# gabrielspmoreira/chameleon_recsys

Hardware: NVIDIA H100
Metric: NAR train interactions/sec (higher is better)
Workload: dtype f32 (wgmma: bf16x3 (error-compensated) forward, single-pass TF32 backward; fp32 accumulate)

## Files before the change

### chameleon_recsys_b200/_lib.py

```python
from __future__ import annotations

import ctypes as C
import os
from typing import Optional

HERE = os.path.dirname(os.path.abspath(__file__))
LIB_PATH = os.path.join(HERE, 'libnar_b200.so')

NAR_MAX_SEGMENTS = 24
NAR_MAX_SRC = 16
NAR_MAX_COLS = 1024

ACT_NONE, ACT_LEAKY, ACT_TANH = 0, 1, 2


class NarError(RuntimeError):
    pass


class Segment(C.Structure):
    _fields_ = [('kind', C.c_int32), ('col', C.c_int32), ('width', C.c_int32), ('card', C.c_int32),
                ('src', C.c_int32), ('ld', C.c_int32), ('table', C.c_void_p), ('grad', C.c_void_p)]


# ... 51 lines not shown


class NoveltyReg(C.Structure):
    _fields_ = [('factor', C.c_float), ('log_base', C.c_float), ('pop_norm', C.c_void_p), ('cand_ids', C.c_void_p),
                ('loss_nov', C.c_void_p)]


class GemmEpilogue(C.Structure):
    _fields_ = [('bias', C.c_void_p), ('act', C.c_int32), ('dact', C.c_int32), ('aux', C.c_void_p),
                ('ld_aux', C.c_int64), ('accumulate', C.c_int32), ('split_k', C.c_int32),
                ('precision', C.c_int32), ('b_lo', C.c_void_p), ('b_bf16', C.c_void_p), ('ld_bf16', C.c_int64),
                ('a_scale', C.c_void_p), ('ld_a_scale', C.c_int64), ('a_scale_group', C.c_int64),
                ('pred', C.c_void_p), ('d_pred', C.c_void_p), ('ld_pred', C.c_int64), ('pred_group', C.c_int64),
                ('d_bias', C.c_void_p), ('car_pp', C.c_void_p), ('car_pc', C.c_void_p), ('car_pi', C.c_void_p), ('car_pos_idx', C.c_void_p),
                ('car_neg_uidx', C.c_void_p), ('car_dpp', C.c_void_p), ('car_dpc', C.c_void_p), ('car_dpi', C.c_void_p),
                ('ld_car', C.c_int64), ('car_k', C.c_int64)]


_lib: Optional[C.CDLL] = None

i64, i32, f32, vp, u64, u32 = C.c_int64, C.c_int32, C.c_float, C.c_void_p, C.c_uint64, C.c_uint32

_SIGNATURES = {
    'nar_abi_version': (C.c_int, []),
    'nar_abi_struct_size': (C.c_int, [C.c_int]),
    'nar_status_string': (C.c_char_p, [C.c_int]),
    'nar_ctx_create': (C.c_int, [C.c_int, C.POINTER(vp)]),
    'nar_ctx_destroy': (C.c_int, [vp]),
    'nar_gather_features': (C.c_int, [vp, C.POINTER(FeaturePlanC), vp, vp, C.POINTER(RowLayout), vp, vp, vp, vp]),
    'nar_gather_features_bwd': (C.c_int, [vp, C.POINTER(FeaturePlanC), vp, vp, C.POINTER(RowLayout), vp, vp, vp, vp, vp, vp]),
    'nar_build_base_rows': (C.c_int, [vp, i64, vp, vp, vp, vp, i64, vp, i64, vp, vp, vp]),
# ... 120 lines not shown
```

### chameleon_recsys_b200/csrc/gemm_wgmma.cu

```cuda
#include "common.cuh"
#include <cuda_bf16.h>
#include <stdlib.h>
#include <string.h>
#include <type_traits>

namespace nar {
namespace gemm {

constexpr int BM = 128;
constexpr int BN = 128;
constexpr int BK = 32;
constexpr int TILE_BYTES = 128 * BK * 4;
constexpr int NUM_THREADS = 256;
constexpr int EPI_LD = BN + 4;

constexpr int EXT_SCALE_SMEM = 1, EXT_SCALE_GMEM = 2, EXT_PROD_BWD = 3, EXT_CAR_BWD = 4, EXT_TRANS_D = 5;
constexpr int SC_ROWS_K = 32, SC_ROWS_MN = 8;
constexpr int SC_BYTES = 4096;
static_assert(SC_ROWS_K * BK * 4 == SC_BYTES && SC_ROWS_MN * BM * 4 == SC_BYTES, "a_scale slice per stage");

template <int MODE, bool B_MN, int SC = 0> struct Cfg {
  static constexpr bool SPLIT3 = MODE == 1 || MODE == 2;
  static constexpr bool BLO = MODE == 2;
  static constexpr bool PREP = B_MN || SPLIT3;
  static constexpr bool PREP_TILES = SPLIT3;
  static constexpr int STAGE_BYTES = TILE_BYTES * (BLO ? 3 : 2);
  static constexpr int CTAS_PER_SM = PREP_TILES ? 1 : 2;
  static constexpr int STAGES = (BLO || !PREP_TILES) ? 3 : 4;
  static constexpr int PREP_TILE_BYTES = PREP_TILES ? TILE_BYTES * 2 : 0;
  static constexpr int PREP_BYTES = 2 * PREP_TILE_BYTES;
  static constexpr int SC_OFF = STAGES * STAGE_BYTES + PREP_BYTES;
  static constexpr int BAR_OFF = SC_OFF + STAGES * SC;
  static constexpr int SMEM_BYTES = BAR_OFF + 64 + 1024;
  static_assert(STAGES * STAGE_BYTES >= BM * EPI_LD * 4, "the epilogue stages the accumulators in the operand ring");
  static_assert(SMEM_BYTES <= 227 * 1024, "227 KB of shared memory per block");
  static_assert(CTAS_PER_SM * (SMEM_BYTES + 1024) <= 228 * 1024, "228 KB of shared memory per SM (1 KB reserved per block)");
};

struct Params {
  int64_t M, N, K;
  float* D; int64_t ldd;
  const float* bias;
  const float* aux; int64_t ld_aux;
  int act, dact, accumulate;
  int k_tiles_per_split;
  int n_tiles;
  const float* a_scale; int64_t ld_a_scale, a_rows, a_cols; uint32_t group;
  const float* pred; float* d_pred; float* d_bias; int64_t ld_pred, n_pos; int pos_per_tile;
  const float *car_pp, *car_pc, *car_pi; const int32_t *car_pos_idx, *car_neg_uidx;
// ... 26 lines not shown

__device__ __forceinline__ void tma_load_2d(uint32_t smem_dst, const CUtensorMap* map, uint64_t* bar, int c0, int c1) {
  asm volatile(
      "cp.async.bulk.tensor.2d.shared::cluster.global.mbarrier::complete_tx::bytes [%0], [%1, {%3, %4}], [%2];"
      ::"r"(smem_dst), "l"(reinterpret_cast<uint64_t>(map)), "r"(smem_u32(bar)), "r"(c0), "r"(c1)
      : "memory");
}
__device__ __forceinline__ void tma_prefetch_desc(const CUtensorMap* map) {
  asm volatile("prefetch.tensormap [%0];" ::"l"(reinterpret_cast<uint64_t>(map)) : "memory");
}

__device__ __forceinline__ void wgmma_fence() { asm volatile("wgmma.fence.sync.aligned;" ::: "memory"); }
__device__ __forceinline__ void wgmma_commit() { asm volatile("wgmma.commit_group.sync.aligned;" ::: "memory"); }
template <int N>
__device__ __forceinline__ void wgmma_wait() { asm volatile("wgmma.wait_group.sync.aligned %0;" ::"n"(N) : "memory"); }
__device__ __forceinline__ void fence_acc(float (&d)[64]) {
#pragma unroll
  for (int i = 0; i < 64; ++i) asm volatile("" : "+f"(d[i])::"memory");
}

__device__ __forceinline__ void wgmma_tf32(float (&d)[64], const uint32_t (&a)[4], uint64_t bdesc) {
  asm volatile(
      "{\n\t.reg .pred p;\n\tsetp.ne.b32 p, 1, 0;\n\t"
      "wgmma.mma_async.sync.aligned.m64n128k8.f32.tf32.tf32 "
      "{%0, %1, %2, %3, %4, %5, %6, %7, %8, %9, %10, %11, %12, %13, %14, %15, "
      "%16, %17, %18, %19, %20, %21, %22, %23, %24, %25, %26, %27, %28, %29, %30, %31, "
      "%32, %33, %34, %35, %36, %37, %38, %39, %40, %41, %42, %43, %44, %45, %46, %47, "
      "%48, %49, %50, %51, %52, %53, %54, %55, %56, %57, %58, %59, %60, %61, %62, %63}, "
      "{%64, %65, %66, %67}, %68, p, 1, 1;\n\t}"
      : "+f"(d[0]), "+f"(d[1]), "+f"(d[2]), "+f"(d[3]), "+f"(d[4]), "+f"(d[5]), "+f"(d[6]), "+f"(d[7]),
        "+f"(d[8]), "+f"(d[9]), "+f"(d[10]), "+f"(d[11]), "+f"(d[12]), "+f"(d[13]), "+f"(d[14]), "+f"(d[15]),
        "+f"(d[16]), "+f"(d[17]), "+f"(d[18]), "+f"(d[19]), "+f"(d[20]), "+f"(d[21]), "+f"(d[22]), "+f"(d[23]),
        "+f"(d[24]), "+f"(d[25]), "+f"(d[26]), "+f"(d[27]), "+f"(d[28]), "+f"(d[29]), "+f"(d[30]), "+f"(d[31]),
// ... 9 lines not shown
      "{\n\t.reg .pred p;\n\tsetp.ne.b32 p, 1, 0;\n\t"
      "wgmma.mma_async.sync.aligned.m64n128k16.f32.bf16.bf16 "
      "{%0, %1, %2, %3, %4, %5, %6, %7, %8, %9, %10, %11, %12, %13, %14, %15, "
      "%16, %17, %18, %19, %20, %21, %22, %23, %24, %25, %26, %27, %28, %29, %30, %31, "
      "%32, %33, %34, %35, %36, %37, %38, %39, %40, %41, %42, %43, %44, %45, %46, %47, "
      "%48, %49, %50, %51, %52, %53, %54, %55, %56, %57, %58, %59, %60, %61, %62, %63}, "
      "{%64, %65, %66, %67}, %68, p, 1, 1, 0;\n\t}"
      : "+f"(d[0]), "+f"(d[1]), "+f"(d[2]), "+f"(d[3]), "+f"(d[4]), "+f"(d[5]), "+f"(d[6]), "+f"(d[7]),
        "+f"(d[8]), "+f"(d[9]), "+f"(d[10]), "+f"(d[11]), "+f"(d[12]), "+f"(d[13]), "+f"(d[14]), "+f"(d[15]),
        "+f"(d[16]), "+f"(d[17]), "+f"(d[18]), "+f"(d[19]), "+f"(d[20]), "+f"(d[21]), "+f"(d[22]), "+f"(d[23]),
        "+f"(d[24]), "+f"(d[25]), "+f"(d[26]), "+f"(d[27]), "+f"(d[28]), "+f"(d[29]), "+f"(d[30]), "+f"(d[31]),
        "+f"(d[32]), "+f"(d[33]), "+f"(d[34]), "+f"(d[35]), "+f"(d[36]), "+f"(d[37]), "+f"(d[38]), "+f"(d[39]),
        "+f"(d[40]), "+f"(d[41]), "+f"(d[42]), "+f"(d[43]), "+f"(d[44]), "+f"(d[45]), "+f"(d[46]), "+f"(d[47]),
        "+f"(d[48]), "+f"(d[49]), "+f"(d[50]), "+f"(d[51]), "+f"(d[52]), "+f"(d[53]), "+f"(d[54]), "+f"(d[55]),
        "+f"(d[56]), "+f"(d[57]), "+f"(d[58]), "+f"(d[59]), "+f"(d[60]), "+f"(d[61]), "+f"(d[62]), "+f"(d[63])
      : "r"(a[0]), "r"(a[1]), "r"(a[2]), "r"(a[3]), "l"(bdesc)
      : "memory");
}

__device__ __forceinline__ uint64_t make_desc(uint32_t saddr) {
  return (uint64_t)((saddr & 0x3FFFFu) >> 4) | (1ull << 16) | ((uint64_t)(1024u >> 4) << 32) | (1ull << 62);
}

__device__ __forceinline__ uint32_t tf32_hi_bits(uint32_t x) { return x & 0xFFFFE000u; }

__device__ __forceinline__ void split_bf16x2(float a, float b, uint32_t& hi, uint32_t& lo) {
  const __nv_bfloat162 h = __floats2bfloat162_rn(a, b);
  const float2 hf = __bfloat1622float2(h);
  const __nv_bfloat162 l = __floats2bfloat162_rn(a - hf.x, b - hf.y);
  hi = *reinterpret_cast<const uint32_t*>(&h);
// ... 273 lines not shown
    for (int r = 1; r < r_end - r_beg; ++r) acc += v[r * EPI_LD];
    atomicAdd(p.car_dpc + l * ld + colc, acc);
  }
}

template <bool MN_MAJOR>
__device__ __forceinline__ void load_operand(uint32_t dst, const CUtensorMap* map, uint64_t* bar, int mn0, int k_elem) {
  if (!MN_MAJOR) {
    tma_load_2d(dst, map, bar, k_elem, mn0);
  } else {
#pragma unroll
    for (int i = 0; i < 4; ++i) tma_load_2d(dst + i * 4096, map, bar, mn0 + i * 32, k_elem);
  }
}

template <bool A_MN, bool B_MN, int MODE, int EXT>
__global__ void __launch_bounds__(NUM_THREADS, (Cfg<MODE, B_MN>::CTAS_PER_SM))
gemm_kernel(const __grid_constant__ CUtensorMap tmap_a, const __grid_constant__ CUtensorMap tmap_b,
            const __grid_constant__ CUtensorMap tmap_x, const Params p) {
  constexpr bool SC_SMEM = EXT == EXT_SCALE_SMEM, SC_GMEM = EXT == EXT_SCALE_GMEM, SCALE = SC_SMEM || SC_GMEM;
  constexpr bool PROD_BWD = EXT == EXT_PROD_BWD, CAR_BWD = EXT == EXT_CAR_BWD, TRANS_D = EXT == EXT_TRANS_D;
  using C = Cfg<MODE, B_MN, SC_SMEM ? SC_BYTES : 0>;
  constexpr bool BF16 = MODE == 4;
  static_assert(!BF16 || !B_MN, "bf16x3: A fp32 of either major, B the transposed (K-major) bf16 plane");
  static_assert(!SCALE || (BF16 && !A_MN) || (MODE == 0 && A_MN && B_MN), "A scale: bf16x3 (K-major A), or single-pass TF32 weight gradient");
  static_assert(!TRANS_D || ((MODE == 0 || MODE == 1) && A_MN && !B_MN), "transposed D: TF32 / 3xTF32, A MN-major, B K-major");
  static_assert(!PROD_BWD || (MODE == 0 && !A_MN && !B_MN), "product backward: single-pass TF32, K-major operands");
  static_assert(!CAR_BWD || ((MODE == 0 || MODE == 1) && !A_MN && !B_MN), "CAR backward: TF32 / 3xTF32, K-major operands");
  static_assert(!CAR_BWD || C::STAGES * C::STAGE_BYTES >= (BM * EPI_LD + 2 * BM) * 4, "CAR backward: row slots behind the staged rows");
  extern __shared__ uint8_t smem_raw[];
  uint8_t* smem = smem_raw + ((1024u - (smem_u32(smem_raw) & 1023u)) & 1023u);
  uint8_t* prep = smem + C::STAGES * C::STAGE_BYTES;
  uint64_t* full = reinterpret_cast<uint64_t*>(smem + C::BAR_OFF);

  const int tid = threadIdx.x;
  const int n_blk = (int)(blockIdx.x % p.n_tiles), m_blk = (int)(blockIdx.x / p.n_tiles);
  const int k_tiles_total = (int)((p.K + BK - 1) / BK);
  const int kt0 = blockIdx.y * p.k_tiles_per_split;
  const int num_kt = min(kt0 + p.k_tiles_per_split, k_tiles_total) - kt0;
  const int m0 = PROD_BWD ? m_blk * p.pos_per_tile * (int)p.group : m_blk * BM;

  if (tid == 0) {
    tma_prefetch_desc(&tmap_a);
    tma_prefetch_desc(&tmap_b);
    if (C::BLO || SC_SMEM) tma_prefetch_desc(&tmap_x);
    for (int s = 0; s < C::STAGES; ++s) mbar_init(&full[s], 1);
    fence_barrier_init();
  }
  __syncthreads();

  auto issue = [&](int kt) {
    const int s = kt % C::STAGES;
    uint64_t* bar = &full[s];
    mbar_expect_tx(bar, C::STAGE_BYTES + (SC_SMEM ? SC_BYTES : 0));
    const uint32_t a_dst = smem_u32(smem + s * C::STAGE_BYTES);
    const uint32_t b_dst = a_dst + TILE_BYTES;
    const int k_elem = (kt0 + kt) * BK;
    load_operand<A_MN>(a_dst, &tmap_a, bar, m0, k_elem);
    if (BF16) {
      tma_load_2d(b_dst, &tmap_b, bar, (kt0 + kt) * 64, n_blk * BN);
    } else {
      load_operand<B_MN>(b_dst, &tmap_b, bar, n_blk * BN, k_elem);
      if (C::BLO) load_operand<B_MN>(b_dst + TILE_BYTES, &tmap_x, bar, n_blk * BN, k_elem);
    }
    if (SC_SMEM) {
      const uint32_t sc_dst = smem_u32(smem + C::SC_OFF + s * SC_BYTES);
      if (A_MN) tma_load_2d(sc_dst, &tmap_x, bar, m0, (int)((uint32_t)k_elem / p.group));
      else tma_load_2d(sc_dst, &tmap_x, bar, k_elem, (int)((uint32_t)m0 / p.group));
    }
  };
  if (tid == 0)
    for (int kt = 0; kt < C::STAGES - 1 && kt < num_kt; ++kt) issue(kt);
  int32_t car_l = -1, car_u = -1;
  if (CAR_BWD) car_bwd_row(p, m0, tid, car_l, car_u);

  const int warp = tid >> 5, lane = tid & 31, g = lane >> 2, t = lane & 3;
  const int r0 = warp * 16 + g;
  float acc[64];
#pragma unroll
  for (int i = 0; i < 64; ++i) acc[i] = 0.f;
  uint32_t a[2][4][4], alo[2][4][4];
  uint32_t ahi16[2][2][4], alo16[2][2][4];
  uint32_t a_off[4];
#pragma unroll
  for (int q = 0; q < 4; ++q)
    a_off[q] = BF16 ? tile_off<true>(r0 + (q >> 1) * 8, 2 * t + (q & 1)) : tile_off<A_MN>(r0 + (q & 1) * 8, t + (q >> 1) * 4);
  const uint32_t sc0 = smem_u32(smem + C::SC_OFF);

  auto k_tile = [&](const int kt, auto buf_tag) {
    constexpr int BUF = decltype(buf_tag)::value;
    const int s = kt % C::STAGES;
    const int k_elem = (kt0 + kt) * BK;
    const uint32_t sc_s = (uint32_t)s * SC_BYTES;
    mbar_wait(&full[s], (uint32_t)(kt / C::STAGES) & 1u);
    const uint8_t* sa = smem + s * C::STAGE_BYTES;
    if (SC_GMEM) {
      scale_tile_gmem<A_MN>(smem + s * C::STAGE_BYTES, p, m0, k_elem, tid);
      __syncthreads();
    }
    uint8_t* sb = smem + s * C::STAGE_BYTES + TILE_BYTES;
    uint8_t* pb = C::PREP_TILES ? prep + BUF * C::PREP_TILE_BYTES : sb;
    if (C::PREP) {
      prep_b<B_MN, MODE>(sb, sb + TILE_BYTES, pb, pb + TILE_BYTES, tid);
      fence_proxy_async_smem();
      __syncthreads();
    }
    const uint32_t b_hi = smem_u32(pb);
    const uint32_t b_lo = b_hi + TILE_BYTES;
    if (BF16) {
      uint32_t sc_r[2] = {0u, 0u};
      if (SC_SMEM)
#pragma unroll
        for (int h = 0; h < 2; ++h)
          sc_r[h] = sc0 + sc_s + ((uint32_t)(m0 + r0 + 8 * h) / p.group - (uint32_t)m0 / p.group) * (BK * 4) + 8 * t;
      uint32_t (&ahi)[2][4] = ahi16[BUF];
// ... 84 lines not shown
    for (; kt + 1 < num_kt; kt += 2) {
      k_tile(kt, std::integral_constant<int, 0>());
      k_tile(kt + 1, std::integral_constant<int, 1>());
    }
    if (kt < num_kt) k_tile(kt, std::integral_constant<int, 0>());
  }
  wgmma_wait<0>();
  fence_acc(acc);
  __syncthreads();

  float* stage = reinterpret_cast<float*>(smem);
  int32_t* s_l = reinterpret_cast<int32_t*>(stage + BM * EPI_LD);
  int32_t* s_u = s_l + BM;
  if (CAR_BWD && tid < BM) { s_l[tid] = car_l; s_u[tid] = car_u; }
#pragma unroll
  for (int j = 0; j < 16; ++j) {
    const int c = 8 * j + 2 * t;
    if (TRANS_D) {
      stage[c * EPI_LD + r0] = acc[4 * j]; stage[(c + 1) * EPI_LD + r0] = acc[4 * j + 1];
      stage[c * EPI_LD + r0 + 8] = acc[4 * j + 2]; stage[(c + 1) * EPI_LD + r0 + 8] = acc[4 * j + 3];
    } else {
      *reinterpret_cast<float2*>(stage + r0 * EPI_LD + c) = make_float2(acc[4 * j], acc[4 * j + 1]);
      *reinterpret_cast<float2*>(stage + (r0 + 8) * EPI_LD + c) = make_float2(acc[4 * j + 2], acc[4 * j + 3]);
    }
  }
  __syncthreads();
  if (PROD_BWD) {
    prod_bwd_epilogue<(C::STAGES * C::STAGE_BYTES - BM * EPI_LD * 4) / (BN * 4)>(p, stage, m_blk, n_blk, tid);
    return;
  }
  if (CAR_BWD) {
    car_bwd_epilogue(p, stage, s_l, s_u, m0, n_blk, tid);
    return;
  }
  if (TRANS_D) {
    const int64_t col = (int64_t)m0 + lane * 4;
    if (col >= p.M) return;
    for (int it = 0; it < BN / 8; ++it) {
      const int nl = it * 8 + warp;
      const int64_t row = (int64_t)n_blk * BN + nl;
      if (row >= p.N) break;
      const float4 v = *reinterpret_cast<const float4*>(stage + nl * EPI_LD + lane * 4);
      float* d = p.D + row * p.ldd + col;
      if (col + 4 <= p.M) {
        if (p.accumulate) atomicAdd(reinterpret_cast<float4*>(d), v);
        else *reinterpret_cast<float4*>(d) = v;
      } else {
        const float e[4] = {v.x, v.y, v.z, v.w};
#pragma unroll
        for (int j = 0; j < 3; ++j)
          if (col + j < p.M) { if (p.accumulate) atomicAdd(d + j, e[j]); else d[j] = e[j]; }
      }
    }
    return;
  }
  const int c4 = lane * 4;
  const int64_t col = (int64_t)n_blk * BN + c4;
  if (col >= p.N) return;
  for (int it = 0; it < BM / 8; ++it) {
    const int rl = it * 8 + warp;
    const int64_t row = (int64_t)m0 + rl;
    if (row >= p.M) break;
    const float4 v = *reinterpret_cast<const float4*>(stage + rl * EPI_LD + c4);
    float4 av = make_float4(0.f, 0.f, 0.f, 0.f);
    if (p.dact && col + 4 <= p.N) av = *reinterpret_cast<const float4*>(p.aux + row * p.ld_aux + col);
    epilogue_store4(p, v, row, col, av);
  }
}

typedef CUresult (*EncodeTiledFn)(CUtensorMap*, CUtensorMapDataType, cuuint32_t, void*, const cuuint64_t*,
                                  const cuuint64_t*, const cuuint32_t*, const cuuint32_t*, CUtensorMapInterleave,
                                  CUtensorMapSwizzle, CUtensorMapL2promotion, CUtensorMapFloatOOBfill);

static int make_operand_map(const nar_ctx* ctx, CUtensorMap* map, const float* ptr, int64_t mn, int64_t k, int64_t ld, bool kmajor) {
  if ((reinterpret_cast<uintptr_t>(ptr) & 15u) != 0 || (ld & 3) != 0 || ld <= 0) return NAR_ERR_INVALID;
  cuuint64_t dims[2]; cuuint64_t strides[1]; cuuint32_t box[2]; cuuint32_t estr[2] = {1, 1};
  if (kmajor) { dims[0] = (cuuint64_t)k; dims[1] = (cuuint64_t)mn; box[0] = BK; box[1] = 128; }
  else        { dims[0] = (cuuint64_t)mn; dims[1] = (cuuint64_t)k; box[0] = 32; box[1] = BK; }
  strides[0] = (cuuint64_t)ld * 4;
  CUresult r = reinterpret_cast<EncodeTiledFn>(ctx->encode_tiled)(
      map, CU_TENSOR_MAP_DATA_TYPE_FLOAT32, 2, const_cast<float*>(ptr), dims, strides, box, estr,
      CU_TENSOR_MAP_INTERLEAVE_NONE, CU_TENSOR_MAP_SWIZZLE_128B, CU_TENSOR_MAP_L2_PROMOTION_L2_256B,
      CU_TENSOR_MAP_FLOAT_OOB_FILL_NONE);
  return r == CUDA_SUCCESS ? NAR_OK : NAR_ERR_INVALID;
}

static int make_bf16_plane_map(const nar_ctx* ctx, CUtensorMap* map, const void* ptr, int64_t n_rows, int64_t k_tiles, int64_t ld) {
  if ((reinterpret_cast<uintptr_t>(ptr) & 15u) != 0 || (ld & 7) != 0 || ld < k_tiles * 64) return NAR_ERR_INVALID;
  cuuint64_t dims[2] = {(cuuint64_t)(k_tiles * 64), (cuuint64_t)n_rows};
  cuuint64_t strides[1] = {(cuuint64_t)ld * 2};
  cuuint32_t box[2] = {64, 128};
  cuuint32_t estr[2] = {1, 1};
  CUresult r = reinterpret_cast<EncodeTiledFn>(ctx->encode_tiled)(
      map, CU_TENSOR_MAP_DATA_TYPE_BFLOAT16, 2, const_cast<void*>(ptr), dims, strides, box, estr, CU_TENSOR_MAP_INTERLEAVE_NONE,
      CU_TENSOR_MAP_SWIZZLE_128B, CU_TENSOR_MAP_L2_PROMOTION_L2_256B, CU_TENSOR_MAP_FLOAT_OOB_FILL_NONE);
  return r == CUDA_SUCCESS ? NAR_OK : NAR_ERR_INVALID;
}

struct PackDesc { const float* W; uint16_t* out; int K, N, ldw, ld_out; };
constexpr int MAX_PACK = 32;
constexpr int PACK_MAX_BLOCKS = 2 * 132;

__global__ void __launch_bounds__(256)
pack_bf16x3_kernel(const PackDesc* __restrict__ descs) {
  __shared__ float tile[32][33];
  const PackDesc d = descs[blockIdx.y];
// ... 20 lines not shown
    }
  }
}

static int make_scale_map(const nar_ctx* ctx, CUtensorMap* map, const float* ptr, int64_t n_groups, int64_t cols, int64_t ld, bool a_mn) {
  cuuint64_t dims[2] = {(cuuint64_t)cols, (cuuint64_t)n_groups};
  cuuint64_t strides[1] = {(cuuint64_t)ld * 4};
  cuuint32_t box[2] = {a_mn ? (cuuint32_t)BM : (cuuint32_t)BK, a_mn ? (cuuint32_t)SC_ROWS_MN : (cuuint32_t)SC_ROWS_K};
  cuuint32_t estr[2] = {1, 1};
  CUresult r = reinterpret_cast<EncodeTiledFn>(ctx->encode_tiled)(
      map, CU_TENSOR_MAP_DATA_TYPE_FLOAT32, 2, const_cast<float*>(ptr), dims, strides, box, estr, CU_TENSOR_MAP_INTERLEAVE_NONE,
      CU_TENSOR_MAP_SWIZZLE_NONE, CU_TENSOR_MAP_L2_PROMOTION_L2_128B, CU_TENSOR_MAP_FLOAT_OOB_FILL_NONE);
  return r == CUDA_SUCCESS ? NAR_OK : NAR_ERR_INVALID;
}

template <bool A_MN, bool B_MN, int MODE, int EXT = 0>
static int launch(const CUtensorMap& ta, const CUtensorMap& tb, const CUtensorMap& tbl, const Params& p, dim3 grid, cudaStream_t st) {
  auto kern = gemm_kernel<A_MN, B_MN, MODE, EXT>;
  constexpr int smem = Cfg<MODE, B_MN, EXT == EXT_SCALE_SMEM ? SC_BYTES : 0>::SMEM_BYTES;
  static bool attr_set = false;
  if (!attr_set) {
    NAR_CHECK_CUDA(cudaFuncSetAttribute(kern, cudaFuncAttributeMaxDynamicSharedMemorySize, smem));
    NAR_CHECK_CUDA(cudaFuncSetAttribute(kern, cudaFuncAttributePreferredSharedMemoryCarveout, cudaSharedmemCarveoutMaxShared));
    attr_set = true;
  }
  kern<<<grid, NUM_THREADS, smem, st>>>(ta, tb, tbl, p);
  NAR_LAUNCH_CHECK();
  return NAR_OK;
}

template <int MODE>
static int ctas_per_sm(bool b_mn) { return b_mn ? Cfg<MODE, true>::CTAS_PER_SM : Cfg<MODE, false>::CTAS_PER_SM; }

}
}

extern "C" int nar_pack_bf16x3(const float* const* W, void* const* out, const int32_t* K, const int32_t* N, const int32_t* ldw,
                               const int32_t* ld_out, int n, void* descs_dev, void* stream) {
  using namespace nar::gemm;
  if (!W || !out || !K || !N || !ldw || !ld_out || !descs_dev || n <= 0 || n > MAX_PACK) return NAR_ERR_INVALID;
  PackDesc h[MAX_PACK];
// ... 56 lines not shown
    return NAR_ERR_INVALID;
  }
  if (car_bwd) {
    const int64_t kk = epi->car_k, ld = epi->ld_car;
    auto al16 = [](const void* q) { return q && (reinterpret_cast<uintptr_t>(q) & 15u) == 0; };
    if ((mode != 0 && mode != 1) || !a_kmajor || !b_kmajor || epi->accumulate || epi->split_k > 1 || epi->bias || epi->act ||
        epi->aux || scale || prod_bwd) return NAR_ERR_INVALID;
    if (kk < 1 || kk > 0x7fffffffLL - 1 || M > 0x7fffffffLL - BM || M % (kk + 1) != 0 || (N & 3) != 0 || ld < N || (ld & 3) != 0)
      return NAR_ERR_INVALID;
    if (!al16(epi->car_pp) || !al16(epi->car_pc) || !al16(epi->car_pi) || !al16(epi->car_dpp) || !al16(epi->car_dpc) ||
        !al16(epi->car_dpi) || !epi->car_pos_idx || !epi->car_neg_uidx) return NAR_ERR_INVALID;
  } else if (epi->car_pc || epi->car_pi || epi->car_pos_idx || epi->car_neg_uidx || epi->car_dpp || epi->car_dpc || epi->car_dpi ||
             epi->ld_car != 0 || epi->car_k != 0) {
    return NAR_ERR_INVALID;
  }
  const int64_t pos_per_tile = prod_bwd ? BM / epi->pred_group : 0, n_pos = prod_bwd ? M / epi->pred_group : 0;
  const int64_t n_tiles = (N + BN - 1) / BN, m_tiles = prod_bwd ? (n_pos + pos_per_tile - 1) / pos_per_tile : (M + BM - 1) / BM;
  if (n_tiles * m_tiles > 0x7fffffffLL) return NAR_ERR_UNSUPPORTED;
  const int k_tiles = (int)((K + BK - 1) / BK);
  const bool amn = !a_kmajor, bmn = !b_kmajor;
  int split = epi->split_k;
  if (split <= 0) {
    split = 1;
    if (epi->accumulate && !epi->bias && !epi->act) {
      const int per_sm = mode == 0 ? ctas_per_sm<0>(bmn) : (mode == 1 ? ctas_per_sm<1>(bmn) : ctas_per_sm<2>(bmn));
      const int64_t fit = (int64_t)per_sm * ctx->sm_count / (n_tiles * m_tiles);
      const int64_t cap = k_tiles / 8 > 1 ? k_tiles / 8 : 1;
      split = (int)(fit < cap ? fit : cap);
      if (split < 1) split = 1;
    }
  }
  if (split > k_tiles) split = k_tiles;
  if (split > 1 && !epi->accumulate) return NAR_ERR_INVALID;
  int per = (k_tiles + split - 1) / split;
  split = (k_tiles + per - 1) / per;
  CUtensorMap ta, tb;
  int rc = make_operand_map(ctx, &ta, A, M, K, lda, a_kmajor != 0);
  if (rc) return rc;
  if (bf16) rc = make_bf16_plane_map(ctx, &tb, epi->b_bf16, N, k_tiles, epi->ld_bf16);
  else rc = make_operand_map(ctx, &tb, B, N, K, ldb, b_kmajor != 0);
  if (rc) return rc;
  CUtensorMap tbl = tb;
  if (blo) {
    rc = make_operand_map(ctx, &tbl, epi->b_lo, N, K, ldb, b_kmajor != 0);
    if (rc) return rc;
  }
  Params p;
  p.M = M; p.N = N; p.K = K; p.D = D; p.ldd = ldd; p.bias = epi->bias; p.aux = epi->aux; p.ld_aux = epi->ld_aux;
  p.act = epi->act; p.dact = epi->dact; p.accumulate = epi->accumulate; p.k_tiles_per_split = per;
  p.n_tiles = (int)n_tiles;
  p.a_scale = epi->a_scale; p.ld_a_scale = epi->ld_a_scale; p.a_rows = a_rows; p.a_cols = a_cols;
  p.group = (uint32_t)(scale ? epi->a_scale_group : (prod_bwd ? epi->pred_group : 1));
  p.pred = epi->pred; p.d_pred = epi->d_pred; p.d_bias = epi->d_bias; p.ld_pred = epi->ld_pred; p.n_pos = n_pos; p.pos_per_tile = (int)pos_per_tile;
  p.car_pp = epi->car_pp; p.car_pc = epi->car_pc; p.car_pi = epi->car_pi; p.car_pos_idx = epi->car_pos_idx;
  p.car_neg_uidx = epi->car_neg_uidx; p.car_dpp = epi->car_dpp; p.car_dpc = epi->car_dpc; p.car_dpi = epi->car_dpi;
  p.ld_car = epi->ld_car; p.car_k = (int)epi->car_k;
  dim3 grid((unsigned)(n_tiles * m_tiles), (unsigned)split, 1);
  cudaStream_t st = as_stream(stream);
  if (scale) {
    const int64_t span = (a_kmajor ? BM - 1 : BK - 1) / epi->a_scale_group + 2;
    if (span <= (a_kmajor ? SC_ROWS_K : SC_ROWS_MN)) {
      rc = make_scale_map(ctx, &tbl, epi->a_scale, (a_rows + epi->a_scale_group - 1) / epi->a_scale_group, a_cols, epi->ld_a_scale,
                          !a_kmajor);
      if (rc) return rc;
      if (mode == 4) return launch<false, false, 4, EXT_SCALE_SMEM>(ta, tb, tbl, p, grid, st);
      return launch<true, true, 0, EXT_SCALE_SMEM>(ta, tb, tbl, p, grid, st);
    }
    if (mode == 4) return launch<false, false, 4, EXT_SCALE_GMEM>(ta, tb, tbl, p, grid, st);
    return launch<true, true, 0, EXT_SCALE_GMEM>(ta, tb, tbl, p, grid, st);
  }
  if (prod_bwd) return launch<false, false, 0, EXT_PROD_BWD>(ta, tb, tbl, p, grid, st);
  if (car_bwd) {
    if (mode == 0) return launch<false, false, 0, EXT_CAR_BWD>(ta, tb, tbl, p, grid, st);
// ... 33 lines not shown
```

### chameleon_recsys_b200/ops.py

```python
from __future__ import annotations

import ctypes as C
from typing import Optional

import torch

from . import _lib
from ._lib import ACT_LEAKY, ACT_NONE, ACT_TANH, Context, FeaturePlanC, GemmEpilogue, NarError, check

_ctx: dict = {}
LAUNCHES = 0


def context(device: Optional[int] = None) -> Context:
    if device is None:
        device = torch.cuda.current_device()
    if device not in _ctx:
        _ctx[device] = Context(device)
    return _ctx[device]


_STREAM_OVERRIDE: Optional[int] = None


# ... 21 lines not shown


def _p(t: Optional[torch.Tensor]) -> C.c_void_p:
    return C.c_void_p(0 if t is None else t.data_ptr())


def _chk_f32(*ts):
    for t in ts:
        if t is not None:
            assert t.is_cuda and t.dtype == torch.float32, (t.device, t.dtype)


def gemm(A: torch.Tensor, B: torch.Tensor, D: torch.Tensor, M: int, N: int, K: int, *, a_kmajor=True, b_kmajor=True,
         lda=None, ldb=None, ldd=None, bias=None, act=ACT_NONE, dact=ACT_NONE, aux=None, ld_aux=None,
         accumulate=False, split_k=1, precision=3, b_lo=None, b_bf16=None, ld_bf16=0, a_scale=None, a_scale_group=0,
         pred=None, d_pred=None, pred_group=0, d_bias=None, car=None, trans_d=False):
    global LAUNCHES
    LAUNCHES += 1
    """D[M,N] = epilogue(sum_k A(m,k) B(n,k)); see nar_gemm_tf32.  a_scale / pred / d_pred: row strides from the tensors.
    d_bias: += the column sums of D (with pred only).
    car: dict(pp, pc, pi, pos_idx, neg_uidx, dpp, dpc, dpi, k) for the CAR layer-1 backward epilogue (D = None; ld_car from
    pp).  trans_d: D stored transposed, D[n*ldd + m] (nar_gemm_tf32_dt)."""
    _chk_f32(A, B, D, bias, aux, a_scale, pred, d_pred, d_bias)
    lda = A.stride(0) if lda is None else lda
    ldb = (B.stride(0) if B is not None else 0) if ldb is None else ldb
    ldd = (D.stride(0) if D is not None else 0) if ldd is None else ldd
    epi = GemmEpilogue(_p(bias), act, dact, _p(aux), (aux.stride(0) if (aux is not None and ld_aux is None) else (ld_aux or 0)),
                       1 if accumulate else 0, int(split_k), int(precision), _p(b_lo), _p(b_bf16), int(ld_bf16),
                       _p(a_scale), a_scale.stride(0) if a_scale is not None else 0, int(a_scale_group),
                       _p(pred), _p(d_pred), pred.stride(0) if pred is not None else 0, int(pred_group), _p(d_bias))
    if car is not None:
        _chk_f32(car['pp'], car['pc'], car['pi'], car['dpp'], car['dpc'], car['dpi'])
        assert car['pos_idx'].dtype == torch.int32 and car['neg_uidx'].dtype == torch.int32
        for f in ('pp', 'pc', 'pi', 'pos_idx', 'neg_uidx', 'dpp', 'dpc', 'dpi'):
            setattr(epi, 'car_' + f, _p(car[f]))
        epi.ld_car, epi.car_k = car['pp'].stride(0), int(car['k'])
    ctx = context()
    fn = 'nar_gemm_tf32_dt' if trans_d else 'nar_gemm_tf32'
    check(getattr(ctx.lib, fn)(ctx.handle, M, N, K, _p(A), lda, 1 if a_kmajor else 0, _p(B), ldb, 1 if b_kmajor else 0,
                               _p(D), ldd, C.byref(epi), _stream()), fn)


_PACK_SCRATCH: dict = {}


def pack_bf16x3(W: torch.Tensor, K: int, N: int) -> torch.Tensor:
    global LAUNCHES
    LAUNCHES += 1
    ld_out = (K + 31) // 32 * 64
    out = torch.zeros(N, ld_out, dtype=torch.bfloat16, device=W.device)
    dev = W.device.index
# ... 237 lines not shown
```

### include/nar_b200.h

```cpp
#ifndef NAR_B200_H
#define NAR_B200_H

#include <stdint.h>

#ifdef __cplusplus
extern "C" {
#endif

#define NAR_ABI_VERSION 3

typedef enum {
  NAR_OK = 0,
  NAR_ERR_INVALID = -1,
  NAR_ERR_UNSUPPORTED = -2,
  NAR_ERR_NO_DEVICE = -3,
  NAR_ERR_WORKSPACE = -4
} nar_status;

typedef struct nar_ctx nar_ctx;

int  nar_abi_version(void);
int  nar_abi_struct_size(int which);
const char* nar_status_string(int status);
int  nar_ctx_create(int device, nar_ctx** out);
// ... 95 lines not shown
  const float* pred;
  float* d_pred;
  int64_t ld_pred;
  int64_t pred_group;
  float* d_bias;
  const float* car_pp;
  const float* car_pc;
  const float* car_pi;
  const int32_t* car_pos_idx;
  const int32_t* car_neg_uidx;
  float* car_dpp;
  float* car_dpc;
  float* car_dpi;
  int64_t ld_car;
  int64_t car_k;
} nar_gemm_epilogue;

int nar_pack_bf16x3(const float* const* W , void* const* out , const int32_t* K, const int32_t* N,
                    const int32_t* ldw, const int32_t* ld_out, int n, void* descs_dev, void* stream);

int nar_gemm_tf32(nar_ctx* ctx, int64_t M, int64_t N, int64_t K,
                  const float* A, int64_t lda, int a_kmajor,
                  const float* B, int64_t ldb, int b_kmajor,
                  float* D, int64_t ldd, const nar_gemm_epilogue* epi , void* stream);
int nar_gemm_tf32_dt(nar_ctx* ctx, int64_t M, int64_t N, int64_t K,
                     const float* A, int64_t lda, int a_kmajor,
                     const float* B, int64_t ldb, int b_kmajor,
                     float* D, int64_t ldd, const nar_gemm_epilogue* epi , void* stream);

int nar_ugrnn_fwd(nar_ctx* ctx, const float* gx , const float* Wh ,
// ... 204 lines not shown
```

Before: 309,200.

## Add 64x64 wgmma tile variant for small GEMMs that underfill the SMs

Adds a 64x64 tile configuration (one warpgroup, 6-stage ring, m64n64 wgmma for TF32 and bf16) to the GEMM kernel. The library picks it automatically when the 128x128 grid would have fewer tiles than SMs, so plain K-major products launch more CTAs and fill the device. The cost is less operand reuse per tile and one more kernel instantiation. A new epilogue field can force either tile size.

```diff
diff --git a/chameleon_recsys_b200/_lib.py b/chameleon_recsys_b200/_lib.py
--- a/chameleon_recsys_b200/_lib.py
+++ b/chameleon_recsys_b200/_lib.py
@@ -89,7 +89,7 @@
                 ('pred', C.c_void_p), ('d_pred', C.c_void_p), ('ld_pred', C.c_int64), ('pred_group', C.c_int64),
                 ('d_bias', C.c_void_p), ('car_pp', C.c_void_p), ('car_pc', C.c_void_p), ('car_pi', C.c_void_p), ('car_pos_idx', C.c_void_p),
                 ('car_neg_uidx', C.c_void_p), ('car_dpp', C.c_void_p), ('car_dpc', C.c_void_p), ('car_dpi', C.c_void_p),
-                ('ld_car', C.c_int64), ('car_k', C.c_int64)]
+                ('ld_car', C.c_int64), ('car_k', C.c_int64), ('tile', C.c_int32)]
 
 
 _lib: Optional[C.CDLL] = None
diff --git a/chameleon_recsys_b200/csrc/gemm_wgmma.cu b/chameleon_recsys_b200/csrc/gemm_wgmma.cu
--- a/chameleon_recsys_b200/csrc/gemm_wgmma.cu
+++ b/chameleon_recsys_b200/csrc/gemm_wgmma.cu
@@ -19,20 +19,25 @@
 constexpr int SC_BYTES = 4096;
 static_assert(SC_ROWS_K * BK * 4 == SC_BYTES && SC_ROWS_MN * BM * 4 == SC_BYTES, "a_scale slice per stage");
 
-template <int MODE, bool B_MN, int SC = 0> struct Cfg {
+template <int MODE, bool B_MN, int SC = 0, bool SMALL = false> struct Cfg {
   static constexpr bool SPLIT3 = MODE == 1 || MODE == 2;
   static constexpr bool BLO = MODE == 2;
   static constexpr bool PREP = B_MN || SPLIT3;
   static constexpr bool PREP_TILES = SPLIT3;
-  static constexpr int STAGE_BYTES = TILE_BYTES * (BLO ? 3 : 2);
-  static constexpr int CTAS_PER_SM = PREP_TILES ? 1 : 2;
-  static constexpr int STAGES = (BLO || !PREP_TILES) ? 3 : 4;
+  static_assert(!SMALL || ((MODE == 0 || MODE == 4) && !B_MN && SC == 0), "64 x 64 tile: single-pass TF32 / bf16x3, K-major B");
+  static constexpr int TBM = SMALL ? 64 : BM, TBN = SMALL ? 64 : BN;
+  static constexpr int THREADS = SMALL ? 128 : NUM_THREADS;
+  static constexpr int A_BYTES = TBM * BK * 4;
+  static constexpr int EPI_LD = TBN + 4;
+  static constexpr int STAGE_BYTES = SMALL ? (TBM + TBN) * BK * 4 : TILE_BYTES * (BLO ? 3 : 2);
+  static constexpr int CTAS_PER_SM = SMALL ? 2 : (PREP_TILES ? 1 : 2);
+  static constexpr int STAGES = SMALL ? 6 : (BLO || !PREP_TILES) ? 3 : 4;
   static constexpr int PREP_TILE_BYTES = PREP_TILES ? TILE_BYTES * 2 : 0;
   static constexpr int PREP_BYTES = 2 * PREP_TILE_BYTES;
   static constexpr int SC_OFF = STAGES * STAGE_BYTES + PREP_BYTES;
   static constexpr int BAR_OFF = SC_OFF + STAGES * SC;
   static constexpr int SMEM_BYTES = BAR_OFF + 64 + 1024;
-  static_assert(STAGES * STAGE_BYTES >= BM * EPI_LD * 4, "the epilogue stages the accumulators in the operand ring");
+  static_assert(STAGES * STAGE_BYTES >= TBM * EPI_LD * 4, "the epilogue stages the accumulators in the operand ring");
   static_assert(SMEM_BYTES <= 227 * 1024, "227 KB of shared memory per block");
   static_assert(CTAS_PER_SM * (SMEM_BYTES + 1024) <= 228 * 1024, "228 KB of shared memory per SM (1 KB reserved per block)");
 };
@@ -89,9 +94,10 @@
 __device__ __forceinline__ void wgmma_commit() { asm volatile("wgmma.commit_group.sync.aligned;" ::: "memory"); }
 template <int N>
 __device__ __forceinline__ void wgmma_wait() { asm volatile("wgmma.wait_group.sync.aligned %0;" ::"n"(N) : "memory"); }
-__device__ __forceinline__ void fence_acc(float (&d)[64]) {
-#pragma unroll
-  for (int i = 0; i < 64; ++i) asm volatile("" : "+f"(d[i])::"memory");
+template <int N>
+__device__ __forceinline__ void fence_acc(float (&d)[N]) {
+#pragma unroll
+  for (int i = 0; i < N; ++i) asm volatile("" : "+f"(d[i])::"memory");
 }
 
 __device__ __forceinline__ void wgmma_tf32(float (&d)[64], const uint32_t (&a)[4], uint64_t bdesc) {
@@ -131,6 +137,35 @@
         "+f"(d[40]), "+f"(d[41]), "+f"(d[42]), "+f"(d[43]), "+f"(d[44]), "+f"(d[45]), "+f"(d[46]), "+f"(d[47]),
         "+f"(d[48]), "+f"(d[49]), "+f"(d[50]), "+f"(d[51]), "+f"(d[52]), "+f"(d[53]), "+f"(d[54]), "+f"(d[55]),
         "+f"(d[56]), "+f"(d[57]), "+f"(d[58]), "+f"(d[59]), "+f"(d[60]), "+f"(d[61]), "+f"(d[62]), "+f"(d[63])
+      : "r"(a[0]), "r"(a[1]), "r"(a[2]), "r"(a[3]), "l"(bdesc)
+      : "memory");
+}
+
+__device__ __forceinline__ void wgmma_tf32(float (&d)[32], const uint32_t (&a)[4], uint64_t bdesc) {
+  asm volatile(
+      "{\n\t.reg .pred p;\n\tsetp.ne.b32 p, 1, 0;\n\t"
+      "wgmma.mma_async.sync.aligned.m64n64k8.f32.tf32.tf32 "
+      "{%0, %1, %2, %3, %4, %5, %6, %7, %8, %9, %10, %11, %12, %13, %14, %15, "
+      "%16, %17, %18, %19, %20, %21, %22, %23, %24, %25, %26, %27, %28, %29, %30, %31}, "
+      "{%32, %33, %34, %35}, %36, p, 1, 1;\n\t}"
+      : "+f"(d[0]), "+f"(d[1]), "+f"(d[2]), "+f"(d[3]), "+f"(d[4]), "+f"(d[5]), "+f"(d[6]), "+f"(d[7]),
+        "+f"(d[8]), "+f"(d[9]), "+f"(d[10]), "+f"(d[11]), "+f"(d[12]), "+f"(d[13]), "+f"(d[14]), "+f"(d[15]),
+        "+f"(d[16]), "+f"(d[17]), "+f"(d[18]), "+f"(d[19]), "+f"(d[20]), "+f"(d[21]), "+f"(d[22]), "+f"(d[23]),
+        "+f"(d[24]), "+f"(d[25]), "+f"(d[26]), "+f"(d[27]), "+f"(d[28]), "+f"(d[29]), "+f"(d[30]), "+f"(d[31])
+      : "r"(a[0]), "r"(a[1]), "r"(a[2]), "r"(a[3]), "l"(bdesc)
+      : "memory");
+}
+__device__ __forceinline__ void wgmma_bf16(float (&d)[32], const uint32_t (&a)[4], uint64_t bdesc) {
+  asm volatile(
+      "{\n\t.reg .pred p;\n\tsetp.ne.b32 p, 1, 0;\n\t"
+      "wgmma.mma_async.sync.aligned.m64n64k16.f32.bf16.bf16 "
+      "{%0, %1, %2, %3, %4, %5, %6, %7, %8, %9, %10, %11, %12, %13, %14, %15, "
+      "%16, %17, %18, %19, %20, %21, %22, %23, %24, %25, %26, %27, %28, %29, %30, %31}, "
+      "{%32, %33, %34, %35}, %36, p, 1, 1, 0;\n\t}"
+      : "+f"(d[0]), "+f"(d[1]), "+f"(d[2]), "+f"(d[3]), "+f"(d[4]), "+f"(d[5]), "+f"(d[6]), "+f"(d[7]),
+        "+f"(d[8]), "+f"(d[9]), "+f"(d[10]), "+f"(d[11]), "+f"(d[12]), "+f"(d[13]), "+f"(d[14]), "+f"(d[15]),
+        "+f"(d[16]), "+f"(d[17]), "+f"(d[18]), "+f"(d[19]), "+f"(d[20]), "+f"(d[21]), "+f"(d[22]), "+f"(d[23]),
+        "+f"(d[24]), "+f"(d[25]), "+f"(d[26]), "+f"(d[27]), "+f"(d[28]), "+f"(d[29]), "+f"(d[30]), "+f"(d[31])
       : "r"(a[0]), "r"(a[1]), "r"(a[2]), "r"(a[3]), "l"(bdesc)
       : "memory");
 }
@@ -434,14 +469,15 @@
   }
 }
 
-template <bool A_MN, bool B_MN, int MODE, int EXT>
-__global__ void __launch_bounds__(NUM_THREADS, (Cfg<MODE, B_MN>::CTAS_PER_SM))
+template <bool A_MN, bool B_MN, int MODE, int EXT, bool SMALL = false>
+__global__ void __launch_bounds__((Cfg<MODE, B_MN, 0, SMALL>::THREADS), (Cfg<MODE, B_MN, 0, SMALL>::CTAS_PER_SM))
 gemm_kernel(const __grid_constant__ CUtensorMap tmap_a, const __grid_constant__ CUtensorMap tmap_b,
             const __grid_constant__ CUtensorMap tmap_x, const Params p) {
   constexpr bool SC_SMEM = EXT == EXT_SCALE_SMEM, SC_GMEM = EXT == EXT_SCALE_GMEM, SCALE = SC_SMEM || SC_GMEM;
   constexpr bool PROD_BWD = EXT == EXT_PROD_BWD, CAR_BWD = EXT == EXT_CAR_BWD, TRANS_D = EXT == EXT_TRANS_D;
-  using C = Cfg<MODE, B_MN, SC_SMEM ? SC_BYTES : 0>;
+  using C = Cfg<MODE, B_MN, SC_SMEM ? SC_BYTES : 0, SMALL>;
   constexpr bool BF16 = MODE == 4;
+  static_assert(!SMALL || (EXT == 0 && !A_MN), "64 x 64 tile: the plain product, K-major A");
   static_assert(!BF16 || !B_MN, "bf16x3: A fp32 of either major, B the transposed (K-major) bf16 plane");
   static_assert(!SCALE || (BF16 && !A_MN) || (MODE == 0 && A_MN && B_MN), "A scale: bf16x3 (K-major A), or single-pass TF32 weight gradient");
   static_assert(!TRANS_D || ((MODE == 0 || MODE == 1) && A_MN && !B_MN), "transposed D: TF32 / 3xTF32, A MN-major, B K-major");
@@ -458,7 +494,7 @@
   const int k_tiles_total = (int)((p.K + BK - 1) / BK);
   const int kt0 = blockIdx.y * p.k_tiles_per_split;
   const int num_kt = min(kt0 + p.k_tiles_per_split, k_tiles_total) - kt0;
-  const int m0 = PROD_BWD ? m_blk * p.pos_per_tile * (int)p.group : m_blk * BM;
+  const int m0 = PROD_BWD ? m_blk * p.pos_per_tile * (int)p.group : m_blk * C::TBM;
 
   if (tid == 0) {
     tma_prefetch_desc(&tmap_a);
@@ -474,13 +510,13 @@
     uint64_t* bar = &full[s];
     mbar_expect_tx(bar, C::STAGE_BYTES + (SC_SMEM ? SC_BYTES : 0));
     const uint32_t a_dst = smem_u32(smem + s * C::STAGE_BYTES);
-    const uint32_t b_dst = a_dst + TILE_BYTES;
+    const uint32_t b_dst = a_dst + C::A_BYTES;
     const int k_elem = (kt0 + kt) * BK;
     load_operand<A_MN>(a_dst, &tmap_a, bar, m0, k_elem);
     if (BF16) {
-      tma_load_2d(b_dst, &tmap_b, bar, (kt0 + kt) * 64, n_blk * BN);
+      tma_load_2d(b_dst, &tmap_b, bar, (kt0 + kt) * 64, n_blk * C::TBN);
     } else {
-      load_operand<B_MN>(b_dst, &tmap_b, bar, n_blk * BN, k_elem);
+      load_operand<B_MN>(b_dst, &tmap_b, bar, n_blk * C::TBN, k_elem);
       if (C::BLO) load_operand<B_MN>(b_dst + TILE_BYTES, &tmap_x, bar, n_blk * BN, k_elem);
     }
     if (SC_SMEM) {
@@ -496,9 +532,9 @@
 
   const int warp = tid >> 5, lane = tid & 31, g = lane >> 2, t = lane & 3;
   const int r0 = warp * 16 + g;
-  float acc[64];
-#pragma unroll
-  for (int i = 0; i < 64; ++i) acc[i] = 0.f;
+  float acc[C::TBN / 2];
+#pragma unroll
+  for (int i = 0; i < C::TBN / 2; ++i) acc[i] = 0.f;
   uint32_t a[2][4][4], alo[2][4][4];
   uint32_t ahi16[2][2][4], alo16[2][2][4];
   uint32_t a_off[4];
@@ -518,7 +554,7 @@
       scale_tile_gmem<A_MN>(smem + s * C::STAGE_BYTES, p, m0, k_elem, tid);
       __syncthreads();
     }
-    uint8_t* sb = smem + s * C::STAGE_BYTES + TILE_BYTES;
+    uint8_t* sb = smem + s * C::STAGE_BYTES + C::A_BYTES;
     uint8_t* pb = C::PREP_TILES ? prep + BUF * C::PREP_TILE_BYTES : sb;
     if (C::PREP) {
       prep_b<B_MN, MODE>(sb, sb + TILE_BYTES, pb, pb + TILE_BYTES, tid);
@@ -633,22 +669,22 @@
   int32_t* s_u = s_l + BM;
   if (CAR_BWD && tid < BM) { s_l[tid] = car_l; s_u[tid] = car_u; }
 #pragma unroll
-  for (int j = 0; j < 16; ++j) {
+  for (int j = 0; j < C::TBN / 8; ++j) {
     const int c = 8 * j + 2 * t;
     if (TRANS_D) {
       stage[c * EPI_LD + r0] = acc[4 * j]; stage[(c + 1) * EPI_LD + r0] = acc[4 * j + 1];
       stage[c * EPI_LD + r0 + 8] = acc[4 * j + 2]; stage[(c + 1) * EPI_LD + r0 + 8] = acc[4 * j + 3];
     } else {
-      *reinterpret_cast<float2*>(stage + r0 * EPI_LD + c) = make_float2(acc[4 * j], acc[4 * j + 1]);
-      *reinterpret_cast<float2*>(stage + (r0 + 8) * EPI_LD + c) = make_float2(acc[4 * j + 2], acc[4 * j + 3]);
+      *reinterpret_cast<float2*>(stage + r0 * C::EPI_LD + c) = make_float2(acc[4 * j], acc[4 * j + 1]);
+      *reinterpret_cast<float2*>(stage + (r0 + 8) * C::EPI_LD + c) = make_float2(acc[4 * j + 2], acc[4 * j + 3]);
     }
   }
   __syncthreads();
-  if (PROD_BWD) {
+  if constexpr (PROD_BWD) {
     prod_bwd_epilogue<(C::STAGES * C::STAGE_BYTES - BM * EPI_LD * 4) / (BN * 4)>(p, stage, m_blk, n_blk, tid);
     return;
   }
-  if (CAR_BWD) {
+  if constexpr (CAR_BWD) {
     car_bwd_epilogue(p, stage, s_l, s_u, m0, n_blk, tid);
     return;
   }
@@ -673,14 +709,15 @@
     }
     return;
   }
-  const int c4 = lane * 4;
-  const int64_t col = (int64_t)n_blk * BN + c4;
+  constexpr int ROW_THREADS = C::TBN / 4;
+  const int c4 = (tid % ROW_THREADS) * 4;
+  const int64_t col = (int64_t)n_blk * C::TBN + c4;
   if (col >= p.N) return;
-  for (int it = 0; it < BM / 8; ++it) {
-    const int rl = it * 8 + warp;
+  for (int it = 0; it < C::TBM / 8; ++it) {
+    const int rl = it * 8 + tid / ROW_THREADS;
     const int64_t row = (int64_t)m0 + rl;
     if (row >= p.M) break;
-    const float4 v = *reinterpret_cast<const float4*>(stage + rl * EPI_LD + c4);
+    const float4 v = *reinterpret_cast<const float4*>(stage + rl * C::EPI_LD + c4);
     float4 av = make_float4(0.f, 0.f, 0.f, 0.f);
     if (p.dact && col + 4 <= p.N) av = *reinterpret_cast<const float4*>(p.aux + row * p.ld_aux + col);
     epilogue_store4(p, v, row, col, av);
@@ -691,10 +728,11 @@
                                   const cuuint64_t*, const cuuint32_t*, const cuuint32_t*, CUtensorMapInterleave,
                                   CUtensorMapSwizzle, CUtensorMapL2promotion, CUtensorMapFloatOOBfill);
 
-static int make_operand_map(const nar_ctx* ctx, CUtensorMap* map, const float* ptr, int64_t mn, int64_t k, int64_t ld, bool kmajor) {
+static int make_operand_map(const nar_ctx* ctx, CUtensorMap* map, const float* ptr, int64_t mn, int64_t k, int64_t ld, bool kmajor,
+                            int box_mn = 128) {
   if ((reinterpret_cast<uintptr_t>(ptr) & 15u) != 0 || (ld & 3) != 0 || ld <= 0) return NAR_ERR_INVALID;
   cuuint64_t dims[2]; cuuint64_t strides[1]; cuuint32_t box[2]; cuuint32_t estr[2] = {1, 1};
-  if (kmajor) { dims[0] = (cuuint64_t)k; dims[1] = (cuuint64_t)mn; box[0] = BK; box[1] = 128; }
+  if (kmajor) { dims[0] = (cuuint64_t)k; dims[1] = (cuuint64_t)mn; box[0] = BK; box[1] = (cuuint32_t)box_mn; }
   else        { dims[0] = (cuuint64_t)mn; dims[1] = (cuuint64_t)k; box[0] = 32; box[1] = BK; }
   strides[0] = (cuuint64_t)ld * 4;
   CUresult r = reinterpret_cast<EncodeTiledFn>(ctx->encode_tiled)(
@@ -704,11 +742,12 @@
   return r == CUDA_SUCCESS ? NAR_OK : NAR_ERR_INVALID;
 }
 
-static int make_bf16_plane_map(const nar_ctx* ctx, CUtensorMap* map, const void* ptr, int64_t n_rows, int64_t k_tiles, int64_t ld) {
+static int make_bf16_plane_map(const nar_ctx* ctx, CUtensorMap* map, const void* ptr, int64_t n_rows, int64_t k_tiles, int64_t ld,
+                               int box_n) {
   if ((reinterpret_cast<uintptr_t>(ptr) & 15u) != 0 || (ld & 7) != 0 || ld < k_tiles * 64) return NAR_ERR_INVALID;
   cuuint64_t dims[2] = {(cuuint64_t)(k_tiles * 64), (cuuint64_t)n_rows};
   cuuint64_t strides[1] = {(cuuint64_t)ld * 2};
-  cuuint32_t box[2] = {64, 128};
+  cuuint32_t box[2] = {64, (cuuint32_t)box_n};
   cuuint32_t estr[2] = {1, 1};
   CUresult r = reinterpret_cast<EncodeTiledFn>(ctx->encode_tiled)(
       map, CU_TENSOR_MAP_DATA_TYPE_BFLOAT16, 2, const_cast<void*>(ptr), dims, strides, box, estr, CU_TENSOR_MAP_INTERLEAVE_NONE,
@@ -759,17 +798,18 @@
   return r == CUDA_SUCCESS ? NAR_OK : NAR_ERR_INVALID;
 }
 
-template <bool A_MN, bool B_MN, int MODE, int EXT = 0>
+template <bool A_MN, bool B_MN, int MODE, int EXT = 0, bool SMALL = false>
 static int launch(const CUtensorMap& ta, const CUtensorMap& tb, const CUtensorMap& tbl, const Params& p, dim3 grid, cudaStream_t st) {
-  auto kern = gemm_kernel<A_MN, B_MN, MODE, EXT>;
-  constexpr int smem = Cfg<MODE, B_MN, EXT == EXT_SCALE_SMEM ? SC_BYTES : 0>::SMEM_BYTES;
+  auto kern = gemm_kernel<A_MN, B_MN, MODE, EXT, SMALL>;
+  using C = Cfg<MODE, B_MN, EXT == EXT_SCALE_SMEM ? SC_BYTES : 0, SMALL>;
+  constexpr int smem = C::SMEM_BYTES;
   static bool attr_set = false;
   if (!attr_set) {
     NAR_CHECK_CUDA(cudaFuncSetAttribute(kern, cudaFuncAttributeMaxDynamicSharedMemorySize, smem));
     NAR_CHECK_CUDA(cudaFuncSetAttribute(kern, cudaFuncAttributePreferredSharedMemoryCarveout, cudaSharedmemCarveoutMaxShared));
     attr_set = true;
   }
-  kern<<<grid, NUM_THREADS, smem, st>>>(ta, tb, tbl, p);
+  kern<<<grid, C::THREADS, smem, st>>>(ta, tb, tbl, p);
   NAR_LAUNCH_CHECK();
   return NAR_OK;
 }
@@ -856,8 +896,15 @@
              epi->ld_car != 0 || epi->car_k != 0) {
     return NAR_ERR_INVALID;
   }
+  if (epi->tile < 0 || epi->tile > 2) return NAR_ERR_INVALID;
+  const bool small_ok = (mode == 0 || mode == 4) && a_kmajor && (bf16 || b_kmajor) && !epi->accumulate && !scale && !prod_bwd &&
+                        !car_bwd && !trans_d;
+  if (epi->tile == 2 && !small_ok) return NAR_ERR_INVALID;
+  const int64_t grid_128 = ((N + BN - 1) / BN) * ((M + BM - 1) / BM);
+  const bool small = epi->tile == 2 || (epi->tile == 0 && small_ok && grid_128 < ctx->sm_count);
+  const int tbm = small ? 64 : BM, tbn = small ? 64 : BN;
   const int64_t pos_per_tile = prod_bwd ? BM / epi->pred_group : 0, n_pos = prod_bwd ? M / epi->pred_group : 0;
-  const int64_t n_tiles = (N + BN - 1) / BN, m_tiles = prod_bwd ? (n_pos + pos_per_tile - 1) / pos_per_tile : (M + BM - 1) / BM;
+  const int64_t n_tiles = (N + tbn - 1) / tbn, m_tiles = prod_bwd ? (n_pos + pos_per_tile - 1) / pos_per_tile : (M + tbm - 1) / tbm;
   if (n_tiles * m_tiles > 0x7fffffffLL) return NAR_ERR_UNSUPPORTED;
   const int k_tiles = (int)((K + BK - 1) / BK);
   const bool amn = !a_kmajor, bmn = !b_kmajor;
@@ -877,10 +924,10 @@
   int per = (k_tiles + split - 1) / split;
   split = (k_tiles + per - 1) / per;
   CUtensorMap ta, tb;
-  int rc = make_operand_map(ctx, &ta, A, M, K, lda, a_kmajor != 0);
+  int rc = make_operand_map(ctx, &ta, A, M, K, lda, a_kmajor != 0, tbm);
   if (rc) return rc;
-  if (bf16) rc = make_bf16_plane_map(ctx, &tb, epi->b_bf16, N, k_tiles, epi->ld_bf16);
-  else rc = make_operand_map(ctx, &tb, B, N, K, ldb, b_kmajor != 0);
+  if (bf16) rc = make_bf16_plane_map(ctx, &tb, epi->b_bf16, N, k_tiles, epi->ld_bf16, tbn);
+  else rc = make_operand_map(ctx, &tb, B, N, K, ldb, b_kmajor != 0, tbn);
   if (rc) return rc;
   CUtensorMap tbl = tb;
   if (blo) {
@@ -899,6 +946,8 @@
   p.ld_car = epi->ld_car; p.car_k = (int)epi->car_k;
   dim3 grid((unsigned)(n_tiles * m_tiles), (unsigned)split, 1);
   cudaStream_t st = as_stream(stream);
+  if (small)
+    return mode == 4 ? launch<false, false, 4, 0, true>(ta, tb, tbl, p, grid, st) : launch<false, false, 0, 0, true>(ta, tb, tbl, p, grid, st);
   if (scale) {
     const int64_t span = (a_kmajor ? BM - 1 : BK - 1) / epi->a_scale_group + 2;
     if (span <= (a_kmajor ? SC_ROWS_K : SC_ROWS_MN)) {
diff --git a/chameleon_recsys_b200/ops.py b/chameleon_recsys_b200/ops.py
--- a/chameleon_recsys_b200/ops.py
+++ b/chameleon_recsys_b200/ops.py
@@ -59,13 +59,14 @@
 def gemm(A: torch.Tensor, B: torch.Tensor, D: torch.Tensor, M: int, N: int, K: int, *, a_kmajor=True, b_kmajor=True,
          lda=None, ldb=None, ldd=None, bias=None, act=ACT_NONE, dact=ACT_NONE, aux=None, ld_aux=None,
          accumulate=False, split_k=1, precision=3, b_lo=None, b_bf16=None, ld_bf16=0, a_scale=None, a_scale_group=0,
-         pred=None, d_pred=None, pred_group=0, d_bias=None, car=None, trans_d=False):
+         pred=None, d_pred=None, pred_group=0, d_bias=None, car=None, trans_d=False, tile=0):
     global LAUNCHES
     LAUNCHES += 1
     """D[M,N] = epilogue(sum_k A(m,k) B(n,k)); see nar_gemm_tf32.  a_scale / pred / d_pred: row strides from the tensors.
     d_bias: += the column sums of D (with pred only).
     car: dict(pp, pc, pi, pos_idx, neg_uidx, dpp, dpc, dpi, k) for the CAR layer-1 backward epilogue (D = None; ld_car from
-    pp).  trans_d: D stored transposed, D[n*ldd + m] (nar_gemm_tf32_dt)."""
+    pp).  trans_d: D stored transposed, D[n*ldd + m] (nar_gemm_tf32_dt).  tile: 0 = the library's choice, 1 = 128 x 128,
+    2 = 64 x 64 (nar_gemm_epilogue.tile)."""
     _chk_f32(A, B, D, bias, aux, a_scale, pred, d_pred, d_bias)
     lda = A.stride(0) if lda is None else lda
     ldb = (B.stride(0) if B is not None else 0) if ldb is None else ldb
@@ -80,6 +81,7 @@
         for f in ('pp', 'pc', 'pi', 'pos_idx', 'neg_uidx', 'dpp', 'dpc', 'dpi'):
             setattr(epi, 'car_' + f, _p(car[f]))
         epi.ld_car, epi.car_k = car['pp'].stride(0), int(car['k'])
+    epi.tile = int(tile)
     ctx = context()
     fn = 'nar_gemm_tf32_dt' if trans_d else 'nar_gemm_tf32'
     check(getattr(ctx.lib, fn)(ctx.handle, M, N, K, _p(A), lda, 1 if a_kmajor else 0, _p(B), ldb, 1 if b_kmajor else 0,
diff --git a/include/nar_b200.h b/include/nar_b200.h
--- a/include/nar_b200.h
+++ b/include/nar_b200.h
@@ -133,6 +133,7 @@
   float* car_dpi;
   int64_t ld_car;
   int64_t car_k;
+  int32_t tile;
 } nar_gemm_epilogue;
 
 int nar_pack_bf16x3(const float* const* W , void* const* out , const int32_t* K, const int32_t* N,
```

New measurement: 315,900, median of 6. 1.02x the previous value.
